# stdstu12/YUME

Measured on NVIDIA H100. Metric: latent_frames_per_sec, higher is better.
Workload: dtype bf16

## Files before the change

yume_b200/csrc/attention.cu:

```cuda
#include "yb_host.h"
#include "yb_ptx.cuh"

namespace yb {

constexpr int ATT_THREADS = 384;
constexpr int ATT_TILE_BYTES = 128 * 128 * 2;

struct AttParams {
  __nv_bfloat16* out;
  long long ldo;
  int Lq, Lk;
  int nkv;
  int accumulate;
  __nv_bfloat16* out_peers[8];
  int sp_world, sp_rank, sp_Lp;
  float scale_log2;
  int nq, full_units, ns;
  float* ws_o;
  float* ws_ml;
};

template <bool P_SMEM>
struct AttCfg {
  static constexpr int NS = P_SMEM ? 4 : 5;
  static constexpr int Q_OFF = 0;
  static constexpr int P_OFF = ATT_TILE_BYTES;
  static constexpr int KV_OFF = P_SMEM ? 2 * ATT_TILE_BYTES : ATT_TILE_BYTES;
  static constexpr int BAR_OFF = KV_OFF + NS * ATT_TILE_BYTES;
  static constexpr int SMEM_BYTES = BAR_OFF + 256 + 1024;
  static_assert(SMEM_BYTES <= 227 * 1024, "shared memory budget");
};

template <bool P_SMEM>
__global__ void __launch_bounds__(ATT_THREADS, 1)
attention_kernel(const __grid_constant__ CUtensorMap tmQ, const __grid_constant__ CUtensorMap tmK,
                 const __grid_constant__ CUtensorMap tmV, const AttParams p) {
  using Cfg = AttCfg<P_SMEM>;
  constexpr int NS = Cfg::NS;
  extern __shared__ uint8_t smem_raw[];
  uint8_t* smem = reinterpret_cast<uint8_t*>((reinterpret_cast<uintptr_t>(smem_raw) + 1023) & ~uintptr_t(1023));
  uint64_t* q_full = reinterpret_cast<uint64_t*>(smem + Cfg::BAR_OFF);
  uint64_t* q_empty = q_full + 1;
  uint64_t* kv_full = q_empty + 1;
  uint64_t* kv_empty = kv_full + NS;

  const int warp = threadIdx.x >> 5;
  const int lane = threadIdx.x & 31;
  int unit = blockIdx.x, kv_begin = 0, nkv = p.nkv;
  if (static_cast<int>(blockIdx.x) >= p.full_units) {
    const int r = blockIdx.x - p.full_units;
    unit = p.full_units + r / p.ns;
    const int per = (((p.nkv + p.ns - 1) / p.ns) + 1) & ~1;
    kv_begin = (r % p.ns) * per;
    nkv = min(per, p.nkv - kv_begin);
  }
  const int head = unit / p.nq;
  const int q0 = (unit - head * p.nq) * 256;
  const int nx = q0 + 128 < p.Lq ? 2 : 1;

  if (threadIdx.x == 0) {
    tma_prefetch_desc(&tmQ);
    tma_prefetch_desc(&tmK);
    tma_prefetch_desc(&tmV);
    mbar_init(q_full, 1);
    mbar_init(q_empty, 8);
    for (int i = 0; i < NS; ++i) {
      mbar_init(&kv_full[i], 1);
      mbar_init(&kv_empty[i], 8);
    }
    fence_barrier_init();
  }
  __syncthreads();

  if (warp < 4) {
    setmaxnreg_dec<40>();
    if (warp == 0 && lane == 0) {
      int it = 0;
      for (int X = 0; X < nx; ++X) {
        if (X == 1) mbar_wait(q_empty, 0);
        mbar_arrive_expect_tx(q_full, ATT_TILE_BYTES);
        for (int s = 0; s < 2; ++s)
          tma_load_2d(smem + Cfg::Q_OFF + s * 16384, &tmQ, q_full, head * 128 + s * 64, q0 + X * 128);
        for (int jj = 0; jj < 2 * nkv; ++jj, ++it) {
          const int slot = it % NS;
          mbar_wait(&kv_empty[slot], ((it / NS) & 1) ^ 1);
          mbar_arrive_expect_tx(&kv_full[slot], ATT_TILE_BYTES);
          const CUtensorMap* tm = (jj & 1) ? &tmV : &tmK;
          uint8_t* dst = smem + Cfg::KV_OFF + slot * ATT_TILE_BYTES;
          const int j = kv_begin + (jj >> 1);
          tma_load_2d(dst, tm, &kv_full[slot], head * 128, j * 128);
          tma_load_2d(dst + 16384, tm, &kv_full[slot], head * 128 + 64, j * 128);
        }
      }
    }
  } else {
    setmaxnreg_inc<232>();
    const int wg = (warp >> 2) - 1;
    const int q4 = lane >> 2, c2 = 2 * (lane & 3);
    const int row_a = wg * 64 + (warp & 3) * 16 + q4;
    const float sc = p.scale_log2;
    const uint32_t sQ = smem_u32(smem + Cfg::Q_OFF) + wg * 64 * 128;
    const uint32_t sP = smem_u32(smem + Cfg::P_OFF) + wg * 16384;
    int it = 0;
    for (int X = 0; X < nx; ++X) {
      mbar_wait(q_full, X);
      float o[64];
#pragma unroll
      for (int i = 0; i < 64; ++i) o[i] = 0.f;
      float m0 = -INFINITY, m1 = -INFINITY, l0 = 0.f, l1 = 0.f;
      for (int j = 0; j < nkv; ++j, it += 2) {
        const int slot_k = it % NS, slot_v = (it + 1) % NS;
        mbar_wait(&kv_full[slot_k], (it / NS) & 1);
        const uint32_t sK = smem_u32(smem + Cfg::KV_OFF + slot_k * ATT_TILE_BYTES);
        float s[64];
#pragma unroll
        for (int i = 0; i < 64; ++i) s[i] = 0.f;
        wgmma_fence();
#pragma unroll
        for (int kk = 0; kk < 8; ++kk) {
          const uint32_t off = (kk >> 2) * 16384 + (kk & 3) * 32;
          wgmma_ss_acc64<0>(s, make_smem_desc_sw128(sQ + off, 16, 1024), make_smem_desc_sw128(sK + off, 16, 1024), kk != 0);
        }
        wgmma_commit();
        wgmma_wait<0>();
        fence_regs(s);
        __syncwarp();
        if (lane == 0) {
          mbar_arrive(&kv_empty[slot_k]);
          if (j == nkv - 1) mbar_arrive(q_empty);
        }
        const int kv_rem = p.Lk - (kv_begin + j) * 128;
        if (kv_rem < 128) {
#pragma unroll
          for (int i = 0; i < 64; ++i)
            if (8 * (i >> 2) + c2 + (i & 1) >= kv_rem) s[i] = -INFINITY;
        }
        float mx0 = -INFINITY, mx1 = -INFINITY;
#pragma unroll
        for (int g = 0; g < 16; ++g) {
          mx0 = fmaxf(mx0, fmaxf(s[4 * g], s[4 * g + 1]));
          mx1 = fmaxf(mx1, fmaxf(s[4 * g + 2], s[4 * g + 3]));
        }
        mx0 = fmaxf(mx0, __shfl_xor_sync(0xffffffffu, mx0, 1));
        mx0 = fmaxf(mx0, __shfl_xor_sync(0xffffffffu, mx0, 2));
        mx1 = fmaxf(mx1, __shfl_xor_sync(0xffffffffu, mx1, 1));
        mx1 = fmaxf(mx1, __shfl_xor_sync(0xffffffffu, mx1, 2));
        const float mn0 = fmaxf(m0, mx0 * sc), mn1 = fmaxf(m1, mx1 * sc);
        const float al0 = fast_exp2(m0 - mn0), al1 = fast_exp2(m1 - mn1);
        m0 = mn0;
        m1 = mn1;
        l0 *= al0;
        l1 *= al1;
#pragma unroll
        for (int g = 0; g < 16; ++g) {
          o[4 * g] *= al0;
          o[4 * g + 1] *= al0;
          o[4 * g + 2] *= al1;
          o[4 * g + 3] *= al1;
        }
        uint32_t pa[8][4];
#pragma unroll
        for (int kk = 0; kk < 8; ++kk) {
          float e[8];
#pragma unroll
          for (int i = 0; i < 8; ++i) e[i] = fast_exp2(s[8 * kk + i] * sc - ((i & 2) ? m1 : m0));
          l0 += (e[0] + e[1]) + (e[4] + e[5]);
          l1 += (e[2] + e[3]) + (e[6] + e[7]);
          pa[kk][0] = pack_bf16x2(e[0], e[1]);
          pa[kk][1] = pack_bf16x2(e[2], e[3]);
          pa[kk][2] = pack_bf16x2(e[4], e[5]);
          pa[kk][3] = pack_bf16x2(e[6], e[7]);
        }
        if (P_SMEM) {
          const int ra = row_a - wg * 64, rb = ra + 8;
#pragma unroll
          for (int kk = 0; kk < 8; ++kk) {
            uint8_t* slab = smem + Cfg::P_OFF + wg * 16384 + (kk >> 2) * 8192;
            const int k0 = (kk & 3) * 16 + c2, k1 = k0 + 8;
            *reinterpret_cast<uint32_t*>(slab + ra * 128 + (((k0 >> 3) ^ (ra & 7)) << 4) + (k0 & 7) * 2) = pa[kk][0];
            *reinterpret_cast<uint32_t*>(slab + rb * 128 + (((k0 >> 3) ^ (rb & 7)) << 4) + (k0 & 7) * 2) = pa[kk][1];
            *reinterpret_cast<uint32_t*>(slab + ra * 128 + (((k1 >> 3) ^ (ra & 7)) << 4) + (k1 & 7) * 2) = pa[kk][2];
            *reinterpret_cast<uint32_t*>(slab + rb * 128 + (((k1 >> 3) ^ (rb & 7)) << 4) + (k1 & 7) * 2) = pa[kk][3];
          }
          fence_proxy_async_smem();
          named_bar_sync(1 + wg, 128);
        }
        mbar_wait(&kv_full[slot_v], ((it + 1) / NS) & 1);
        const uint32_t sV = smem_u32(smem + Cfg::KV_OFF + slot_v * ATT_TILE_BYTES);
        wgmma_fence();
#pragma unroll
        for (int kk = 0; kk < 8; ++kk) {
          const uint64_t vdesc = make_smem_desc_sw128(sV + kk * 2048, 16384, 1024);
          if (P_SMEM)
            wgmma_ss_acc64<1>(o, make_smem_desc_sw128(sP + (kk >> 2) * 8192 + (kk & 3) * 32, 16, 1024), vdesc, 1u);
          else
            wgmma_rs_n128_tb(o, pa[kk], vdesc, 1u);
        }
        wgmma_commit();
        wgmma_wait<0>();
        fence_regs(o);
        __syncwarp();
        if (lane == 0) mbar_arrive(&kv_empty[slot_v]);
      }
      l0 += __shfl_xor_sync(0xffffffffu, l0, 1);
      l0 += __shfl_xor_sync(0xffffffffu, l0, 2);
      l1 += __shfl_xor_sync(0xffffffffu, l1, 1);
      l1 += __shfl_xor_sync(0xffffffffu, l1, 2);

#pragma unroll
      for (int h = 0; h < 2; ++h) {
        const int row_t = X * 128 + row_a + 8 * h;
        const float m = h ? m1 : m0, l = h ? l1 : l0;
        if (static_cast<int>(blockIdx.x) >= p.full_units) {
          const long long prow = static_cast<long long>(blockIdx.x - p.full_units) * 256 + row_t;
          float* wo = p.ws_o + prow * 128;
#pragma unroll
          for (int g = 0; g < 16; ++g) *reinterpret_cast<float2*>(wo + 8 * g + c2) = make_float2(o[4 * g + 2 * h], o[4 * g + 2 * h + 1]);
          if ((lane & 3) == 0) *reinterpret_cast<float2*>(p.ws_ml + prow * 2) = make_float2(m, l);
          continue;
        }
        const int q_row = q0 + row_t;
        if (q_row >= p.Lq) continue;
        __nv_bfloat16* orow = p.out + static_cast<long long>(q_row) * p.ldo + head * 128;
        if (p.sp_world > 1) {
          const int owner = q_row / p.sp_Lp;
          const int t = q_row - owner * p.sp_Lp;
          if (owner < p.sp_world)
            orow = p.out_peers[owner] + (static_cast<long long>(p.sp_rank) * p.sp_Lp + t) * p.ldo + head * 128;
        }
        const float inv = 1.0f / l;
#pragma unroll
        for (int g = 0; g < 16; ++g) {
          uint32_t* dst = reinterpret_cast<uint32_t*>(orow + 8 * g + c2);
          float v0 = o[4 * g + 2 * h] * inv, v1 = o[4 * g + 2 * h + 1] * inv;
          if (p.accumulate) {
            const float2 prev = __bfloat1622float2(*reinterpret_cast<const __nv_bfloat162*>(dst));
            v0 += prev.x;
            v1 += prev.y;
          }
          *dst = pack_bf16x2(v0, v1);
        }
      }
    }
  }
}

__global__ void __launch_bounds__(256) attention_combine_kernel(const AttParams p, int tail_units) {
  const int gw = blockIdx.x * 8 + (threadIdx.x >> 5);
  const int lane = threadIdx.x & 31;
  if (gw >= tail_units * 256) return;
  const int tu = gw >> 8, r = gw & 255;
  const int unit = p.full_units + tu;
  const int head = unit / p.nq;
  const int q_row = (unit - head * p.nq) * 256 + r;
  if (q_row >= p.Lq) return;
  float M = -INFINITY;
  for (int sgm = 0; sgm < p.ns; ++sgm) M = fmaxf(M, p.ws_ml[((static_cast<long long>(tu) * p.ns + sgm) * 256 + r) * 2]);
  float4 acc = make_float4(0.f, 0.f, 0.f, 0.f);
  float lsum = 0.f;
  for (int sgm = 0; sgm < p.ns; ++sgm) {
    const long long prow = (static_cast<long long>(tu) * p.ns + sgm) * 256 + r;
    const float2 ml = *reinterpret_cast<const float2*>(p.ws_ml + prow * 2);
    const float w = exp2f(ml.x - M);
    const float4 o = *reinterpret_cast<const float4*>(p.ws_o + prow * 128 + lane * 4);
    acc.x += o.x * w; acc.y += o.y * w; acc.z += o.z * w; acc.w += o.w * w;
    lsum += ml.y * w;
  }
  const float inv = 1.0f / lsum;
  __nv_bfloat16* orow = p.out + static_cast<long long>(q_row) * p.ldo + head * 128;
  if (p.sp_world > 1) {
    const int owner = q_row / p.sp_Lp;
    const int t = q_row - owner * p.sp_Lp;
    if (owner < p.sp_world)
      orow = p.out_peers[owner] + (static_cast<long long>(p.sp_rank) * p.sp_Lp + t) * p.ldo + head * 128;
  }
  *reinterpret_cast<uint2*>(orow + lane * 4) = make_uint2(pack_bf16x2(acc.x * inv, acc.y * inv), pack_bf16x2(acc.z * inv, acc.w * inv));
}

static void attention_plan(int units, int nkv, int sms, bool allowed, int force_ns, int* full_units, int* tail, int* ns) {
  *full_units = units;
  *tail = 0;
  *ns = 1;
  if (!allowed || force_ns == 1) return;
  if (force_ns >= 2 && nkv >= 2 * force_ns) {
    *tail = units;
    *ns = force_ns;
  } else if (force_ns == 0 && units > sms && units % sms != 0 && 2 * (units % sms) <= sms && nkv >= 16) {
    *tail = units % sms;
    *ns = sms / *tail < 4 ? sms / *tail : 4;
  }
  while (*ns > 1 && (*ns - 1) * ((((nkv + *ns - 1) / *ns) + 1) & ~1) >= nkv) --*ns;
  if (*ns == 1) *tail = 0;
  *full_units = units - *tail;
}

static size_t split_workspace_bytes(size_t ctas) { return ctas * 256 * 130 * sizeof(float); }

static int g_debug_force_split = 0;

template <bool P_SMEM>
static int launch_attention(const CUtensorMap& tmQ, const CUtensorMap& tmK, const CUtensorMap& tmV,
                            AttParams p, int heads, cudaStream_t stream, int force_ns, void* ws, long long ws_bytes) {
  using Cfg = AttCfg<P_SMEM>;
  auto kern = attention_kernel<P_SMEM>;
  static bool attr_set[kMaxDevices] = {false};
  if (int rc = ensure_dynamic_smem(kern, Cfg::SMEM_BYTES, attr_set, "attention")) return rc;
  if (force_ns == 0 && g_debug_force_split >= 1 && g_debug_force_split <= 4) force_ns = g_debug_force_split;
  p.nq = (p.Lq + 255) / 256;
  const int units = p.nq * heads;
  int tail = 0;
  p.ws_o = p.ws_ml = nullptr;
  const bool allowed = !p.accumulate && ws != nullptr;
  attention_plan(units, p.nkv, sm_count(), allowed, force_ns, &p.full_units, &tail, &p.ns);
  if (tail > 0) {
    const size_t ctas = static_cast<size_t>(tail) * p.ns;
    if (ws_bytes < 0 || static_cast<size_t>(ws_bytes) < split_workspace_bytes(ctas) || (reinterpret_cast<uintptr_t>(ws) & 0xF)) {
      p.full_units = units;
      tail = 0;
      p.ns = 1;
    } else {
      p.ws_o = static_cast<float*>(ws);
      p.ws_ml = p.ws_o + ctas * 256 * 128;
    }
  }
  kern<<<p.full_units + tail * p.ns, ATT_THREADS, Cfg::SMEM_BYTES, stream>>>(tmQ, tmK, tmV, p);
  int rc = check_launch("attention");
  if (rc || tail == 0) return rc;
  attention_combine_kernel<<<tail * 32, 256, 0, stream>>>(p, tail);
  return check_launch("attention_combine");
}

static int dispatch_attention(const void* q, long long ldq, const void* k, long long ldk, const void* v, long long ldv,
                              AttParams p, int heads, cudaStream_t stream, int flags, void* ws, long long ws_bytes) {
  const int force_ns = (flags >> YB_ATT_SPLIT_SHIFT) & 7;
  if (force_ns > 4) return YB_ERR_ARG;
  if ((flags >> YB_ATT_EMU_SHIFT) & 3) return YB_ERR_ARG;
  CUtensorMap tmQ, tmK, tmV;
  const uint64_t cols = static_cast<uint64_t>(heads) * 128;
  int rc = make_tmap_bf16_2d(&tmQ, q, p.Lq, cols, ldq, 128, 64);
  if (rc) return rc;
  rc = make_tmap_bf16_2d(&tmK, k, p.Lk, cols, ldk, 128, 64);
  if (rc) return rc;
  rc = make_tmap_bf16_2d(&tmV, v, p.Lk, cols, ldv, 128, 64);
  if (rc) return rc;
  if (flags & YB_ATT_P_SMEM) return launch_attention<true>(tmQ, tmK, tmV, p, heads, stream, force_ns, ws, ws_bytes);
  return launch_attention<false>(tmQ, tmK, tmV, p, heads, stream, force_ns, ws, ws_bytes);
}

}

extern "C" int yb_debug_force_split(int ns) {
  if (ns < 0 || ns > 4) return YB_ERR_ARG;
  yb::g_debug_force_split = ns;
  return YB_OK;
}

extern "C" int yb_attention_plan(int Lq, int Lk, int heads, int sms, int flags, int* out4) {
  if (Lq <= 0 || Lk <= 0 || heads <= 0 || sms <= 0 || !out4) return YB_ERR_ARG;
  int force_ns = (flags >> YB_ATT_SPLIT_SHIFT) & 7;
  if (force_ns > 4) return YB_ERR_ARG;
  if (force_ns == 0 && yb::g_debug_force_split >= 1) force_ns = yb::g_debug_force_split;
  const int nkv = (Lk + 127) / 128;
  int full_units, tail, ns;
  yb::attention_plan(((Lq + 255) / 256) * heads, nkv, sms, !(flags & YB_ATT_ACCUMULATE), force_ns, &full_units, &tail, &ns);
  out4[0] = full_units;
  out4[1] = tail;
  out4[2] = ns;
  out4[3] = ns > 1 ? ((((nkv + ns - 1) / ns) + 1) & ~1) : nkv;
  return YB_OK;
}

extern "C" long long yb_attention_workspace_bytes(int Lq, int Lk, int heads, int sms, int flags) {
  int plan[4];
  if (yb_attention_plan(Lq, Lk, heads, sms, flags, plan)) return -1;
  return static_cast<long long>(yb::split_workspace_bytes(static_cast<size_t>(plan[1]) * plan[2]));
}

extern "C" int yb_attention_ex(const void* q, long long ldq, const void* k, long long ldk, const void* v,
                               long long ldv, void* out, long long ldo, int Lq, int Lk, int heads, float scale,
                               int flags, void* ws, long long ws_bytes, void* trace, void* stream_) {
  using namespace yb;
  if (!q || !k || !v || !out) return YB_ERR_ARG;
  if (Lq <= 0 || Lk <= 0 || heads <= 0) return YB_ERR_ARG;
  if ((ldo % 8) != 0 || (reinterpret_cast<uintptr_t>(out) & 0xF)) return YB_ERR_ALIGNMENT;
  AttParams p;
  p.out = static_cast<__nv_bfloat16*>(out);
  p.ldo = ldo;
  p.Lq = Lq;
  p.Lk = Lk;
  p.nkv = (Lk + 127) / 128;
  p.accumulate = (flags & YB_ATT_ACCUMULATE) ? 1 : 0;
  (void)trace;
  p.sp_world = 1;
  p.sp_rank = 0;
  p.sp_Lp = 0;
  p.scale_log2 = scale * 1.4426950408889634f;
  return dispatch_attention(q, ldq, k, ldk, v, ldv, p, heads, reinterpret_cast<cudaStream_t>(stream_), flags, ws, ws_bytes);
}

extern "C" int yb_attention(const void* q, long long ldq, const void* k, long long ldk, const void* v, long long ldv,
                            void* out, long long ldo, int Lq, int Lk, int heads, float scale, int flags,
                            void* stream_) {
  return yb_attention_ex(q, ldq, k, ldk, v, ldv, out, ldo, Lq, Lk, heads, scale, flags, nullptr, 0, nullptr, stream_);
}

extern "C" int yb_attention_sp(const void* q, long long ldq, const void* k, long long ldk, const void* v, long long ldv,
                               void* const* out_peers, long long ldo, int Lq, int Lk, int heads, float scale, int world,
                               int rank, int Lp, int flags, void* ws, long long ws_bytes, void* stream_) {
  using namespace yb;
  if (!q || !k || !v || !out_peers || world < 2 || world > 8 || rank < 0 || rank >= world || Lp <= 0) return YB_ERR_ARG;
  if (Lq != world * Lp || Lk <= 0 || Lk > Lq || heads <= 0 || (ldo % 8)) return YB_ERR_ARG;
  if (flags & (YB_ATT_ACCUMULATE | YB_ATT_P_SMEM)) return YB_ERR_ARG;
  AttParams p;
  p.out = static_cast<__nv_bfloat16*>(out_peers[rank]);
  p.ldo = ldo;
  p.Lq = Lq;
  p.Lk = Lk;
  p.nkv = (Lk + 127) / 128;
  p.accumulate = 0;
  p.scale_log2 = scale * 1.4426950408889634f;
  for (int i = 0; i < 8; ++i) p.out_peers[i] = i < world ? static_cast<__nv_bfloat16*>(out_peers[i]) : nullptr;
  p.sp_world = world;
  p.sp_rank = rank;
  p.sp_Lp = Lp;
  return dispatch_attention(q, ldq, k, ldk, v, ldv, p, heads, reinterpret_cast<cudaStream_t>(stream_), flags, ws, ws_bytes);
}
```

yume_b200/csrc/yb_ptx.cuh:

```cuda
#pragma once
#include <cstdint>
#include <cstdio>
#include <cuda.h>
#include <cuda_runtime.h>
#include <cuda_bf16.h>

namespace yb {

__device__ __forceinline__ uint32_t smem_u32(const void* p) {
  return static_cast<uint32_t>(__cvta_generic_to_shared(p));
}

template <int N>
__device__ __forceinline__ void setmaxnreg_inc() {
  asm volatile("setmaxnreg.inc.sync.aligned.u32 %0;\n" ::"n"(N));
}
template <int N>
__device__ __forceinline__ void setmaxnreg_dec() {
  asm volatile("setmaxnreg.dec.sync.aligned.u32 %0;\n" ::"n"(N));
}
__device__ __forceinline__ void named_bar_sync(int id, int count) {
  asm volatile("bar.sync %0, %1;" ::"r"(id), "r"(count) : "memory");
}

__device__ __forceinline__ void mbar_init(uint64_t* bar, uint32_t count) {
  asm volatile("mbarrier.init.shared::cta.b64 [%0], %1;" ::"r"(smem_u32(bar)), "r"(count) : "memory");
}
__device__ __forceinline__ void fence_barrier_init() {
  asm volatile("fence.mbarrier_init.release.cluster;" ::: "memory");
}
__device__ __forceinline__ void fence_proxy_async_smem() {
  asm volatile("fence.proxy.async.shared::cta;" ::: "memory");
}
__device__ __forceinline__ void mbar_arrive_expect_tx(uint64_t* bar, uint32_t bytes) {
  asm volatile("mbarrier.arrive.expect_tx.shared::cta.b64 _, [%0], %1;" ::"r"(smem_u32(bar)), "r"(bytes)
               : "memory");
}
__device__ __forceinline__ void mbar_arrive(uint64_t* bar) {
  asm volatile("mbarrier.arrive.shared::cta.b64 _, [%0];" ::"r"(smem_u32(bar)) : "memory");
}
__device__ __forceinline__ bool mbar_try_wait(uint64_t* bar, uint32_t parity) {
  uint32_t ok;
  asm volatile(
      "{\n\t.reg .pred p;\n\t"
      "mbarrier.try_wait.parity.shared::cta.b64 p, [%1], %2;\n\t"
      "selp.u32 %0, 1, 0, p;\n\t}\n"
      : "=r"(ok)
      : "r"(smem_u32(bar)), "r"(parity)
      : "memory");
  return ok != 0;
}
#ifndef YB_WAIT_LIMIT_CYCLES
#define YB_WAIT_LIMIT_CYCLES 8000000000LL
#endif
__device__ __forceinline__ void mbar_wait(uint64_t* bar, uint32_t parity) {
  if (mbar_try_wait(bar, parity)) return;
  const long long t0 = clock64();
  while (!mbar_try_wait(bar, parity)) {
    if (clock64() - t0 > YB_WAIT_LIMIT_CYCLES) {
#ifdef YB_DEBUG_WAIT
      printf("yb: mbarrier wait timeout block=(%d,%d) thread=%d bar=%u parity=%u\n", blockIdx.x, blockIdx.y,
             threadIdx.x, smem_u32(bar), parity);
#endif
      __trap();
    }
  }
}
__device__ __forceinline__ void mbar_wait_cluster(uint64_t* bar, uint32_t parity) {
  const long long t0 = clock64();
  for (;;) {
    uint32_t ok;
    asm volatile(
        "{\n\t.reg .pred p;\n\t"
        "mbarrier.try_wait.parity.acquire.cluster.shared::cta.b64 p, [%1], %2;\n\t"
        "selp.u32 %0, 1, 0, p;\n\t}\n"
        : "=r"(ok)
        : "r"(smem_u32(bar)), "r"(parity)
        : "memory");
    if (ok) return;
    if (clock64() - t0 > YB_WAIT_LIMIT_CYCLES) __trap();
  }
}

__device__ __forceinline__ uint32_t cluster_ctarank() {
  uint32_t r;
  asm volatile("mov.u32 %0, %%cluster_ctarank;" : "=r"(r));
  return r;
}
__device__ __forceinline__ void cluster_sync_all() {
  asm volatile("barrier.cluster.arrive.release.aligned;\n\tbarrier.cluster.wait.acquire.aligned;" ::: "memory");
}
__device__ __forceinline__ void mbar_arrive_cluster(uint64_t* bar, uint32_t cta) {
  uint32_t remote;
  asm volatile("mapa.shared::cluster.u32 %0, %1, %2;" : "=r"(remote) : "r"(smem_u32(bar)), "r"(cta));
  asm volatile("mbarrier.arrive.release.cluster.shared::cluster.b64 _, [%0];" ::"r"(remote) : "memory");
}

__device__ __forceinline__ void tma_prefetch_desc(const CUtensorMap* tmap) {
  asm volatile("prefetch.tensormap [%0];" ::"l"(reinterpret_cast<uint64_t>(tmap)) : "memory");
}
__device__ __forceinline__ void tma_load_2d(void* smem_dst, const CUtensorMap* tmap, uint64_t* bar, int c0, int c1) {
  asm volatile(
      "cp.async.bulk.tensor.2d.shared::cluster.global.tile.mbarrier::complete_tx::bytes [%0], [%1, {%3, %4}], [%2];"
      ::"r"(smem_u32(smem_dst)), "l"(reinterpret_cast<uint64_t>(tmap)), "r"(smem_u32(bar)), "r"(c0), "r"(c1)
      : "memory");
}
__device__ __forceinline__ void tma_load_2d_multicast(void* smem_dst, const CUtensorMap* tmap, uint64_t* bar, int c0, int c1,
                                                      uint16_t mask) {
  asm volatile(
      "cp.async.bulk.tensor.2d.shared::cluster.global.mbarrier::complete_tx::bytes.multicast::cluster [%0], [%1, {%3, %4}], "
      "[%2], %5;" ::"r"(smem_u32(smem_dst)),
      "l"(reinterpret_cast<uint64_t>(tmap)), "r"(smem_u32(bar)), "r"(c0), "r"(c1), "h"(mask)
      : "memory");
}
__device__ __forceinline__ void tma_load_3d(void* smem_dst, const CUtensorMap* tmap, uint64_t* bar, int c0, int c1,
                                            int c2) {
  asm volatile(
      "cp.async.bulk.tensor.3d.shared::cluster.global.tile.mbarrier::complete_tx::bytes [%0], [%1, {%3, %4, %5}], [%2];"
      ::"r"(smem_u32(smem_dst)), "l"(reinterpret_cast<uint64_t>(tmap)), "r"(smem_u32(bar)), "r"(c0), "r"(c1), "r"(c2)
      : "memory");
}
__device__ __forceinline__ void tma_load_4d(void* smem_dst, const CUtensorMap* tmap, uint64_t* bar, int c0, int c1,
                                            int c2, int c3) {
  asm volatile(
      "cp.async.bulk.tensor.4d.shared::cluster.global.tile.mbarrier::complete_tx::bytes [%0], [%1, {%3, %4, %5, %6}], [%2];"
      ::"r"(smem_u32(smem_dst)), "l"(reinterpret_cast<uint64_t>(tmap)), "r"(smem_u32(bar)), "r"(c0), "r"(c1), "r"(c2),
      "r"(c3)
      : "memory");
}

__device__ __forceinline__ uint64_t make_smem_desc_sw128(uint32_t smem_addr, uint32_t lbo_bytes, uint32_t sbo_bytes) {
  uint64_t d = 0;
  d |= static_cast<uint64_t>((smem_addr & 0x3FFFF) >> 4);
  d |= static_cast<uint64_t>((lbo_bytes >> 4) & 0x3FFF) << 16;
  d |= static_cast<uint64_t>((sbo_bytes >> 4) & 0x3FFF) << 32;
  d |= static_cast<uint64_t>(1) << 62;
  return d;
}
__device__ __forceinline__ void wgmma_fence() { asm volatile("wgmma.fence.sync.aligned;" ::: "memory"); }
__device__ __forceinline__ void wgmma_commit() { asm volatile("wgmma.commit_group.sync.aligned;" ::: "memory"); }
template <int N>
__device__ __forceinline__ void wgmma_wait() {
  asm volatile("wgmma.wait_group.sync.aligned %0;" ::"n"(N) : "memory");
}
template <int R>
__device__ __forceinline__ void fence_regs(float (&d)[R]) {
#pragma unroll
  for (int i = 0; i < R; ++i) asm volatile("" : "+f"(d[i])::"memory");
}

template <int OFF>
__device__ __forceinline__ void wgmma_ss_n64(float (&d)[128], uint64_t adesc, uint64_t bdesc, uint32_t accumulate) {
  asm volatile(
      "{\n\t.reg .pred p;\n\t"
      "setp.ne.b32 p, %34, 0;\n\t"
      "wgmma.mma_async.sync.aligned.m64n64k16.f32.bf16.bf16 {%0, %1, %2, %3, %4, %5, %6, %7, %8, %9, %10, %11, %12, %13, %14, %15, %16, %17, %18, %19, %20, %21, %22, %23, %24, %25, %26, %27, %28, %29, %30, %31}, %32, %33, p, 1, 1, 0, 0;\n\t}\n"
      : "+f"(d[OFF + 0]), "+f"(d[OFF + 1]), "+f"(d[OFF + 2]), "+f"(d[OFF + 3]), "+f"(d[OFF + 4]), "+f"(d[OFF + 5]), "+f"(d[OFF + 6]), "+f"(d[OFF + 7]), "+f"(d[OFF + 8]), "+f"(d[OFF + 9]), "+f"(d[OFF + 10]), "+f"(d[OFF + 11]), "+f"(d[OFF + 12]), "+f"(d[OFF + 13]), "+f"(d[OFF + 14]), "+f"(d[OFF + 15]), "+f"(d[OFF + 16]), "+f"(d[OFF + 17]), "+f"(d[OFF + 18]), "+f"(d[OFF + 19]), "+f"(d[OFF + 20]), "+f"(d[OFF + 21]), "+f"(d[OFF + 22]), "+f"(d[OFF + 23]), "+f"(d[OFF + 24]), "+f"(d[OFF + 25]), "+f"(d[OFF + 26]), "+f"(d[OFF + 27]), "+f"(d[OFF + 28]), "+f"(d[OFF + 29]), "+f"(d[OFF + 30]), "+f"(d[OFF + 31])
      : "l"(adesc), "l"(bdesc), "r"(accumulate));
}
template <int OFF>
__device__ __forceinline__ void wgmma_ss_n128(float (&d)[128], uint64_t adesc, uint64_t bdesc, uint32_t accumulate) {
  asm volatile(
      "{\n\t.reg .pred p;\n\t"
      "setp.ne.b32 p, %66, 0;\n\t"
      "wgmma.mma_async.sync.aligned.m64n128k16.f32.bf16.bf16 {%0, %1, %2, %3, %4, %5, %6, %7, %8, %9, %10, %11, %12, %13, %14, %15, %16, %17, %18, %19, %20, %21, %22, %23, %24, %25, %26, %27, %28, %29, %30, %31, %32, %33, %34, %35, %36, %37, %38, %39, %40, %41, %42, %43, %44, %45, %46, %47, %48, %49, %50, %51, %52, %53, %54, %55, %56, %57, %58, %59, %60, %61, %62, %63}, %64, %65, p, 1, 1, 0, 0;\n\t}\n"
      : "+f"(d[OFF + 0]), "+f"(d[OFF + 1]), "+f"(d[OFF + 2]), "+f"(d[OFF + 3]), "+f"(d[OFF + 4]), "+f"(d[OFF + 5]), "+f"(d[OFF + 6]), "+f"(d[OFF + 7]), "+f"(d[OFF + 8]), "+f"(d[OFF + 9]), "+f"(d[OFF + 10]), "+f"(d[OFF + 11]), "+f"(d[OFF + 12]), "+f"(d[OFF + 13]), "+f"(d[OFF + 14]), "+f"(d[OFF + 15]), "+f"(d[OFF + 16]), "+f"(d[OFF + 17]), "+f"(d[OFF + 18]), "+f"(d[OFF + 19]), "+f"(d[OFF + 20]), "+f"(d[OFF + 21]), "+f"(d[OFF + 22]), "+f"(d[OFF + 23]), "+f"(d[OFF + 24]), "+f"(d[OFF + 25]), "+f"(d[OFF + 26]), "+f"(d[OFF + 27]), "+f"(d[OFF + 28]), "+f"(d[OFF + 29]), "+f"(d[OFF + 30]), "+f"(d[OFF + 31]), "+f"(d[OFF + 32]), "+f"(d[OFF + 33]), "+f"(d[OFF + 34]), "+f"(d[OFF + 35]), "+f"(d[OFF + 36]), "+f"(d[OFF + 37]), "+f"(d[OFF + 38]), "+f"(d[OFF + 39]), "+f"(d[OFF + 40]), "+f"(d[OFF + 41]), "+f"(d[OFF + 42]), "+f"(d[OFF + 43]), "+f"(d[OFF + 44]), "+f"(d[OFF + 45]), "+f"(d[OFF + 46]), "+f"(d[OFF + 47]), "+f"(d[OFF + 48]), "+f"(d[OFF + 49]), "+f"(d[OFF + 50]), "+f"(d[OFF + 51]), "+f"(d[OFF + 52]), "+f"(d[OFF + 53]), "+f"(d[OFF + 54]), "+f"(d[OFF + 55]), "+f"(d[OFF + 56]), "+f"(d[OFF + 57]), "+f"(d[OFF + 58]), "+f"(d[OFF + 59]), "+f"(d[OFF + 60]), "+f"(d[OFF + 61]), "+f"(d[OFF + 62]), "+f"(d[OFF + 63])
      : "l"(adesc), "l"(bdesc), "r"(accumulate));
}
template <int OFF>
__device__ __forceinline__ void wgmma_ss_n256(float (&d)[128], uint64_t adesc, uint64_t bdesc, uint32_t accumulate) {
  asm volatile(
      "{\n\t.reg .pred p;\n\t"
      "setp.ne.b32 p, %130, 0;\n\t"
      "wgmma.mma_async.sync.aligned.m64n256k16.f32.bf16.bf16 {%0, %1, %2, %3, %4, %5, %6, %7, %8, %9, %10, %11, %12, %13, %14, %15, %16, %17, %18, %19, %20, %21, %22, %23, %24, %25, %26, %27, %28, %29, %30, %31, %32, %33, %34, %35, %36, %37, %38, %39, %40, %41, %42, %43, %44, %45, %46, %47, %48, %49, %50, %51, %52, %53, %54, %55, %56, %57, %58, %59, %60, %61, %62, %63, %64, %65, %66, %67, %68, %69, %70, %71, %72, %73, %74, %75, %76, %77, %78, %79, %80, %81, %82, %83, %84, %85, %86, %87, %88, %89, %90, %91, %92, %93, %94, %95, %96, %97, %98, %99, %100, %101, %102, %103, %104, %105, %106, %107, %108, %109, %110, %111, %112, %113, %114, %115, %116, %117, %118, %119, %120, %121, %122, %123, %124, %125, %126, %127}, %128, %129, p, 1, 1, 0, 0;\n\t}\n"
      : "+f"(d[OFF + 0]), "+f"(d[OFF + 1]), "+f"(d[OFF + 2]), "+f"(d[OFF + 3]), "+f"(d[OFF + 4]), "+f"(d[OFF + 5]), "+f"(d[OFF + 6]), "+f"(d[OFF + 7]), "+f"(d[OFF + 8]), "+f"(d[OFF + 9]), "+f"(d[OFF + 10]), "+f"(d[OFF + 11]), "+f"(d[OFF + 12]), "+f"(d[OFF + 13]), "+f"(d[OFF + 14]), "+f"(d[OFF + 15]), "+f"(d[OFF + 16]), "+f"(d[OFF + 17]), "+f"(d[OFF + 18]), "+f"(d[OFF + 19]), "+f"(d[OFF + 20]), "+f"(d[OFF + 21]), "+f"(d[OFF + 22]), "+f"(d[OFF + 23]), "+f"(d[OFF + 24]), "+f"(d[OFF + 25]), "+f"(d[OFF + 26]), "+f"(d[OFF + 27]), "+f"(d[OFF + 28]), "+f"(d[OFF + 29]), "+f"(d[OFF + 30]), "+f"(d[OFF + 31]), "+f"(d[OFF + 32]), "+f"(d[OFF + 33]), "+f"(d[OFF + 34]), "+f"(d[OFF + 35]), "+f"(d[OFF + 36]), "+f"(d[OFF + 37]), "+f"(d[OFF + 38]), "+f"(d[OFF + 39]), "+f"(d[OFF + 40]), "+f"(d[OFF + 41]), "+f"(d[OFF + 42]), "+f"(d[OFF + 43]), "+f"(d[OFF + 44]), "+f"(d[OFF + 45]), "+f"(d[OFF + 46]), "+f"(d[OFF + 47]), "+f"(d[OFF + 48]), "+f"(d[OFF + 49]), "+f"(d[OFF + 50]), "+f"(d[OFF + 51]), "+f"(d[OFF + 52]), "+f"(d[OFF + 53]), "+f"(d[OFF + 54]), "+f"(d[OFF + 55]), "+f"(d[OFF + 56]), "+f"(d[OFF + 57]), "+f"(d[OFF + 58]), "+f"(d[OFF + 59]), "+f"(d[OFF + 60]), "+f"(d[OFF + 61]), "+f"(d[OFF + 62]), "+f"(d[OFF + 63]), "+f"(d[OFF + 64]), "+f"(d[OFF + 65]), "+f"(d[OFF + 66]), "+f"(d[OFF + 67]), "+f"(d[OFF + 68]), "+f"(d[OFF + 69]), "+f"(d[OFF + 70]), "+f"(d[OFF + 71]), "+f"(d[OFF + 72]), "+f"(d[OFF + 73]), "+f"(d[OFF + 74]), "+f"(d[OFF + 75]), "+f"(d[OFF + 76]), "+f"(d[OFF + 77]), "+f"(d[OFF + 78]), "+f"(d[OFF + 79]), "+f"(d[OFF + 80]), "+f"(d[OFF + 81]), "+f"(d[OFF + 82]), "+f"(d[OFF + 83]), "+f"(d[OFF + 84]), "+f"(d[OFF + 85]), "+f"(d[OFF + 86]), "+f"(d[OFF + 87]), "+f"(d[OFF + 88]), "+f"(d[OFF + 89]), "+f"(d[OFF + 90]), "+f"(d[OFF + 91]), "+f"(d[OFF + 92]), "+f"(d[OFF + 93]), "+f"(d[OFF + 94]), "+f"(d[OFF + 95]), "+f"(d[OFF + 96]), "+f"(d[OFF + 97]), "+f"(d[OFF + 98]), "+f"(d[OFF + 99]), "+f"(d[OFF + 100]), "+f"(d[OFF + 101]), "+f"(d[OFF + 102]), "+f"(d[OFF + 103]), "+f"(d[OFF + 104]), "+f"(d[OFF + 105]), "+f"(d[OFF + 106]), "+f"(d[OFF + 107]), "+f"(d[OFF + 108]), "+f"(d[OFF + 109]), "+f"(d[OFF + 110]), "+f"(d[OFF + 111]), "+f"(d[OFF + 112]), "+f"(d[OFF + 113]), "+f"(d[OFF + 114]), "+f"(d[OFF + 115]), "+f"(d[OFF + 116]), "+f"(d[OFF + 117]), "+f"(d[OFF + 118]), "+f"(d[OFF + 119]), "+f"(d[OFF + 120]), "+f"(d[OFF + 121]), "+f"(d[OFF + 122]), "+f"(d[OFF + 123]), "+f"(d[OFF + 124]), "+f"(d[OFF + 125]), "+f"(d[OFF + 126]), "+f"(d[OFF + 127])
      : "l"(adesc), "l"(bdesc), "r"(accumulate));
}
__device__ __forceinline__ void wgmma_rs_n128_tb(float (&d)[64], const uint32_t (&a)[4], uint64_t bdesc, uint32_t accumulate) {
  asm volatile(
      "{\n\t.reg .pred p;\n\t"
      "setp.ne.b32 p, %69, 0;\n\t"
      "wgmma.mma_async.sync.aligned.m64n128k16.f32.bf16.bf16 {%0, %1, %2, %3, %4, %5, %6, %7, %8, %9, %10, %11, %12, %13, %14, %15, %16, %17, %18, %19, %20, %21, %22, %23, %24, %25, %26, %27, %28, %29, %30, %31, %32, %33, %34, %35, %36, %37, %38, %39, %40, %41, %42, %43, %44, %45, %46, %47, %48, %49, %50, %51, %52, %53, %54, %55, %56, %57, %58, %59, %60, %61, %62, %63}, {%64, %65, %66, %67}, %68, p, 1, 1, 1;\n\t}\n"
      : "+f"(d[0]), "+f"(d[1]), "+f"(d[2]), "+f"(d[3]), "+f"(d[4]), "+f"(d[5]), "+f"(d[6]), "+f"(d[7]), "+f"(d[8]), "+f"(d[9]), "+f"(d[10]), "+f"(d[11]), "+f"(d[12]), "+f"(d[13]), "+f"(d[14]), "+f"(d[15]), "+f"(d[16]), "+f"(d[17]), "+f"(d[18]), "+f"(d[19]), "+f"(d[20]), "+f"(d[21]), "+f"(d[22]), "+f"(d[23]), "+f"(d[24]), "+f"(d[25]), "+f"(d[26]), "+f"(d[27]), "+f"(d[28]), "+f"(d[29]), "+f"(d[30]), "+f"(d[31]), "+f"(d[32]), "+f"(d[33]), "+f"(d[34]), "+f"(d[35]), "+f"(d[36]), "+f"(d[37]), "+f"(d[38]), "+f"(d[39]), "+f"(d[40]), "+f"(d[41]), "+f"(d[42]), "+f"(d[43]), "+f"(d[44]), "+f"(d[45]), "+f"(d[46]), "+f"(d[47]), "+f"(d[48]), "+f"(d[49]), "+f"(d[50]), "+f"(d[51]), "+f"(d[52]), "+f"(d[53]), "+f"(d[54]), "+f"(d[55]), "+f"(d[56]), "+f"(d[57]), "+f"(d[58]), "+f"(d[59]), "+f"(d[60]), "+f"(d[61]), "+f"(d[62]), "+f"(d[63])
      : "r"(a[0]), "r"(a[1]), "r"(a[2]), "r"(a[3]), "l"(bdesc), "r"(accumulate));
}
template <int TB>
__device__ __forceinline__ void wgmma_ss_acc64(float (&d)[64], uint64_t adesc, uint64_t bdesc, uint32_t accumulate) {
  asm volatile(
      "{\n\t.reg .pred p;\n\t"
      "setp.ne.b32 p, %66, 0;\n\t"
      "wgmma.mma_async.sync.aligned.m64n128k16.f32.bf16.bf16 {%0, %1, %2, %3, %4, %5, %6, %7, %8, %9, %10, %11, %12, %13, %14, %15, %16, %17, %18, %19, %20, %21, %22, %23, %24, %25, %26, %27, %28, %29, %30, %31, %32, %33, %34, %35, %36, %37, %38, %39, %40, %41, %42, %43, %44, %45, %46, %47, %48, %49, %50, %51, %52, %53, %54, %55, %56, %57, %58, %59, %60, %61, %62, %63}, %64, %65, p, 1, 1, 0, %67;\n\t}\n"
      : "+f"(d[0]), "+f"(d[1]), "+f"(d[2]), "+f"(d[3]), "+f"(d[4]), "+f"(d[5]), "+f"(d[6]), "+f"(d[7]), "+f"(d[8]), "+f"(d[9]), "+f"(d[10]), "+f"(d[11]), "+f"(d[12]), "+f"(d[13]), "+f"(d[14]), "+f"(d[15]), "+f"(d[16]), "+f"(d[17]), "+f"(d[18]), "+f"(d[19]), "+f"(d[20]), "+f"(d[21]), "+f"(d[22]), "+f"(d[23]), "+f"(d[24]), "+f"(d[25]), "+f"(d[26]), "+f"(d[27]), "+f"(d[28]), "+f"(d[29]), "+f"(d[30]), "+f"(d[31]), "+f"(d[32]), "+f"(d[33]), "+f"(d[34]), "+f"(d[35]), "+f"(d[36]), "+f"(d[37]), "+f"(d[38]), "+f"(d[39]), "+f"(d[40]), "+f"(d[41]), "+f"(d[42]), "+f"(d[43]), "+f"(d[44]), "+f"(d[45]), "+f"(d[46]), "+f"(d[47]), "+f"(d[48]), "+f"(d[49]), "+f"(d[50]), "+f"(d[51]), "+f"(d[52]), "+f"(d[53]), "+f"(d[54]), "+f"(d[55]), "+f"(d[56]), "+f"(d[57]), "+f"(d[58]), "+f"(d[59]), "+f"(d[60]), "+f"(d[61]), "+f"(d[62]), "+f"(d[63])
      : "l"(adesc), "l"(bdesc), "r"(accumulate), "n"(TB));
}

__device__ __forceinline__ uint32_t pack_bf16x2(float lo, float hi) {
  __nv_bfloat162 v = __floats2bfloat162_rn(lo, hi);
  return *reinterpret_cast<uint32_t*>(&v);
}
__device__ __forceinline__ float fast_exp2(float x) {
  float y;
  asm volatile("ex2.approx.ftz.f32 %0, %1;" : "=f"(y) : "f"(x));
  return y;
}
__device__ __forceinline__ float fast_tanh(float x) {
  float y;
  asm volatile("tanh.approx.f32 %0, %1;" : "=f"(y) : "f"(x));
  return y;
}
__device__ __forceinline__ float gelu_tanh(float x) {
  const float k0 = 0.7978845608028654f, k1 = 0.044715f;
  float u = k0 * (x + k1 * x * x * x);
  return 0.5f * x * (1.0f + fast_tanh(u));
}

}
```

Baseline: 38.83.

## Overlap softmax with next QK GEMM and ping-pong warpgroups in attention

Restructures the consumer loop of the attention kernel in the FA3 style. The S=QK^T GEMM for block j is issued together with the PV GEMM for block j-1, and the softmax of block j runs while the PV GEMM is still in flight. Named barriers make the two consumer warpgroups take turns issuing WGMMAs, so one warpgroup's softmax overlaps the other's tensor-core work. It also moves the trap out of line in mbar_wait to shrink code, at the cost of more live registers and more complex barrier protocols.

Result: faster. 39.83, median of 6 (+2.6%).

```diff
diff --git a/yume_b200/csrc/attention.cu b/yume_b200/csrc/attention.cu
--- a/yume_b200/csrc/attention.cu
+++ b/yume_b200/csrc/attention.cu
@@ -101,107 +101,155 @@
     const float sc = p.scale_log2;
     const uint32_t sQ = smem_u32(smem + Cfg::Q_OFF) + wg * 64 * 128;
     const uint32_t sP = smem_u32(smem + Cfg::P_OFF) + wg * 16384;
-    int it = 0;
-    for (int X = 0; X < nx; ++X) {
+    float o[64], s[64];
+    uint32_t pa[8][4];
+    float m0 = -INFINITY, m1 = -INFINITY, l0 = 0.f, l1 = 0.f;
+
+    auto kv_wait = [&](int i) { mbar_wait(&kv_full[i % NS], (i / NS) & 1); };
+    auto kv_release = [&](int i) {
+      __syncwarp();
+      if (lane == 0) mbar_arrive(&kv_empty[i % NS]);
+    };
+    auto kv_smem = [&](int i) { return smem_u32(smem + Cfg::KV_OFF + (i % NS) * ATT_TILE_BYTES); };
+    auto issue_s = [&](int i) {
+      const uint32_t sK = kv_smem(i);
+#pragma unroll
+      for (int c = 0; c < 64; ++c) s[c] = 0.f;
+      wgmma_fence();
+#pragma unroll
+      for (int kk = 0; kk < 8; ++kk) {
+        const uint32_t off = (kk >> 2) * 16384 + (kk & 3) * 32;
+        wgmma_ss_acc64<0>(s, make_smem_desc_sw128(sQ + off, 16, 1024), make_smem_desc_sw128(sK + off, 16, 1024), kk != 0);
+      }
+      wgmma_commit();
+    };
+    auto issue_pv = [&](int i) {
+      const uint32_t sV = kv_smem(i);
+      wgmma_fence();
+#pragma unroll
+      for (int kk = 0; kk < 8; ++kk) {
+        const uint64_t vdesc = make_smem_desc_sw128(sV + kk * 2048, 16384, 1024);
+        if (P_SMEM)
+          wgmma_ss_acc64<1>(o, make_smem_desc_sw128(sP + (kk >> 2) * 8192 + (kk & 3) * 32, 16, 1024), vdesc, 1u);
+        else
+          wgmma_rs_n128_tb(o, pa[kk], vdesc, 1u);
+      }
+      wgmma_commit();
+    };
+    auto softmax = [&](int j, float& al0, float& al1) {
+      const int kv_rem = p.Lk - (kv_begin + j) * 128;
+      if (kv_rem < 128) {
+#pragma unroll
+        for (int i = 0; i < 64; ++i)
+          if (8 * (i >> 2) + c2 + (i & 1) >= kv_rem) s[i] = -INFINITY;
+      }
+      float mx0 = -INFINITY, mx1 = -INFINITY;
+#pragma unroll
+      for (int g = 0; g < 16; ++g) {
+        mx0 = fmaxf(mx0, fmaxf(s[4 * g], s[4 * g + 1]));
+        mx1 = fmaxf(mx1, fmaxf(s[4 * g + 2], s[4 * g + 3]));
+      }
+      mx0 = fmaxf(mx0, __shfl_xor_sync(0xffffffffu, mx0, 1));
+      mx0 = fmaxf(mx0, __shfl_xor_sync(0xffffffffu, mx0, 2));
+      mx1 = fmaxf(mx1, __shfl_xor_sync(0xffffffffu, mx1, 1));
+      mx1 = fmaxf(mx1, __shfl_xor_sync(0xffffffffu, mx1, 2));
+      const float mn0 = fmaxf(m0, mx0 * sc), mn1 = fmaxf(m1, mx1 * sc);
+      al0 = fast_exp2(m0 - mn0);
+      al1 = fast_exp2(m1 - mn1);
+      m0 = mn0;
+      m1 = mn1;
+      l0 *= al0;
+      l1 *= al1;
+#pragma unroll
+      for (int kk = 0; kk < 8; ++kk) {
+        float* e = s + 8 * kk;
+#pragma unroll
+        for (int i = 0; i < 8; ++i) e[i] = fast_exp2(e[i] * sc - ((i & 2) ? m1 : m0));
+        l0 += (e[0] + e[1]) + (e[4] + e[5]);
+        l1 += (e[2] + e[3]) + (e[6] + e[7]);
+      }
+    };
+    auto rescale_pack = [&](float al0, float al1) {
+#pragma unroll
+      for (int g = 0; g < 16; ++g) {
+        o[4 * g] *= al0;
+        o[4 * g + 1] *= al0;
+        o[4 * g + 2] *= al1;
+        o[4 * g + 3] *= al1;
+      }
+#pragma unroll
+      for (int kk = 0; kk < 8; ++kk) {
+        const float* e = s + 8 * kk;
+        pa[kk][0] = pack_bf16x2(e[0], e[1]);
+        pa[kk][1] = pack_bf16x2(e[2], e[3]);
+        pa[kk][2] = pack_bf16x2(e[4], e[5]);
+        pa[kk][3] = pack_bf16x2(e[6], e[7]);
+      }
+      if (P_SMEM) {
+        const int ra = row_a - wg * 64, rb = ra + 8;
+#pragma unroll
+        for (int kk = 0; kk < 8; ++kk) {
+          uint8_t* slab = smem + Cfg::P_OFF + wg * 16384 + (kk >> 2) * 8192;
+          const int k0 = (kk & 3) * 16 + c2, k1 = k0 + 8;
+          *reinterpret_cast<uint32_t*>(slab + ra * 128 + (((k0 >> 3) ^ (ra & 7)) << 4) + (k0 & 7) * 2) = pa[kk][0];
+          *reinterpret_cast<uint32_t*>(slab + rb * 128 + (((k0 >> 3) ^ (rb & 7)) << 4) + (k0 & 7) * 2) = pa[kk][1];
+          *reinterpret_cast<uint32_t*>(slab + ra * 128 + (((k1 >> 3) ^ (ra & 7)) << 4) + (k1 & 7) * 2) = pa[kk][2];
+          *reinterpret_cast<uint32_t*>(slab + rb * 128 + (((k1 >> 3) ^ (rb & 7)) << 4) + (k1 & 7) * 2) = pa[kk][3];
+        }
+        fence_proxy_async_smem();
+        named_bar_sync(1 + wg, 128);
+      }
+    };
+    auto turn_wait = [&]() { named_bar_sync(3 + wg, 256); };
+    auto turn_pass = [&](bool last) {
+      if (wg == 0 || !last) named_bar_arrive(4 - wg, 256);
+    };
+
+    if (wg == 1) named_bar_arrive(3, 256);
+    int it0 = 0;
+    for (int X = 0; X < nx; ++X, it0 += 2 * nkv) {
       mbar_wait(q_full, X);
-      float o[64];
 #pragma unroll
       for (int i = 0; i < 64; ++i) o[i] = 0.f;
-      float m0 = -INFINITY, m1 = -INFINITY, l0 = 0.f, l1 = 0.f;
-      for (int j = 0; j < nkv; ++j, it += 2) {
-        const int slot_k = it % NS, slot_v = (it + 1) % NS;
-        mbar_wait(&kv_full[slot_k], (it / NS) & 1);
-        const uint32_t sK = smem_u32(smem + Cfg::KV_OFF + slot_k * ATT_TILE_BYTES);
-        float s[64];
-#pragma unroll
-        for (int i = 0; i < 64; ++i) s[i] = 0.f;
-        wgmma_fence();
-#pragma unroll
-        for (int kk = 0; kk < 8; ++kk) {
-          const uint32_t off = (kk >> 2) * 16384 + (kk & 3) * 32;
-          wgmma_ss_acc64<0>(s, make_smem_desc_sw128(sQ + off, 16, 1024), make_smem_desc_sw128(sK + off, 16, 1024), kk != 0);
-        }
-        wgmma_commit();
-        wgmma_wait<0>();
+      m0 = m1 = -INFINITY;
+      l0 = l1 = 0.f;
+      float al0, al1;
+      kv_wait(it0);
+      turn_wait();
+      issue_s(it0);
+      turn_pass(X == nx - 1 && nkv == 1);
+      wgmma_wait<0>();
+      fence_regs(s);
+      kv_release(it0);
+      if (nkv == 1 && lane == 0) mbar_arrive(q_empty);
+      softmax(0, al0, al1);
+      rescale_pack(al0, al1);
+      for (int j = 1; j < nkv; ++j) {
+        const int ik = it0 + 2 * j;
+        kv_wait(ik);
+        kv_wait(ik - 1);
+        turn_wait();
+        issue_s(ik);
+        issue_pv(ik - 1);
+        turn_pass(X == nx - 1 && j == nkv - 1);
+        wgmma_wait<1>();
         fence_regs(s);
-        __syncwarp();
-        if (lane == 0) {
-          mbar_arrive(&kv_empty[slot_k]);
-          if (j == nkv - 1) mbar_arrive(q_empty);
-        }
-        const int kv_rem = p.Lk - (kv_begin + j) * 128;
-        if (kv_rem < 128) {
-#pragma unroll
-          for (int i = 0; i < 64; ++i)
-            if (8 * (i >> 2) + c2 + (i & 1) >= kv_rem) s[i] = -INFINITY;
-        }
-        float mx0 = -INFINITY, mx1 = -INFINITY;
-#pragma unroll
-        for (int g = 0; g < 16; ++g) {
-          mx0 = fmaxf(mx0, fmaxf(s[4 * g], s[4 * g + 1]));
-          mx1 = fmaxf(mx1, fmaxf(s[4 * g + 2], s[4 * g + 3]));
-        }
-        mx0 = fmaxf(mx0, __shfl_xor_sync(0xffffffffu, mx0, 1));
-        mx0 = fmaxf(mx0, __shfl_xor_sync(0xffffffffu, mx0, 2));
-        mx1 = fmaxf(mx1, __shfl_xor_sync(0xffffffffu, mx1, 1));
-        mx1 = fmaxf(mx1, __shfl_xor_sync(0xffffffffu, mx1, 2));
-        const float mn0 = fmaxf(m0, mx0 * sc), mn1 = fmaxf(m1, mx1 * sc);
-        const float al0 = fast_exp2(m0 - mn0), al1 = fast_exp2(m1 - mn1);
-        m0 = mn0;
-        m1 = mn1;
-        l0 *= al0;
-        l1 *= al1;
-#pragma unroll
-        for (int g = 0; g < 16; ++g) {
-          o[4 * g] *= al0;
-          o[4 * g + 1] *= al0;
-          o[4 * g + 2] *= al1;
-          o[4 * g + 3] *= al1;
-        }
-        uint32_t pa[8][4];
-#pragma unroll
-        for (int kk = 0; kk < 8; ++kk) {
-          float e[8];
-#pragma unroll
-          for (int i = 0; i < 8; ++i) e[i] = fast_exp2(s[8 * kk + i] * sc - ((i & 2) ? m1 : m0));
-          l0 += (e[0] + e[1]) + (e[4] + e[5]);
-          l1 += (e[2] + e[3]) + (e[6] + e[7]);
-          pa[kk][0] = pack_bf16x2(e[0], e[1]);
-          pa[kk][1] = pack_bf16x2(e[2], e[3]);
-          pa[kk][2] = pack_bf16x2(e[4], e[5]);
-          pa[kk][3] = pack_bf16x2(e[6], e[7]);
-        }
-        if (P_SMEM) {
-          const int ra = row_a - wg * 64, rb = ra + 8;
-#pragma unroll
-          for (int kk = 0; kk < 8; ++kk) {
-            uint8_t* slab = smem + Cfg::P_OFF + wg * 16384 + (kk >> 2) * 8192;
-            const int k0 = (kk & 3) * 16 + c2, k1 = k0 + 8;
-            *reinterpret_cast<uint32_t*>(slab + ra * 128 + (((k0 >> 3) ^ (ra & 7)) << 4) + (k0 & 7) * 2) = pa[kk][0];
-            *reinterpret_cast<uint32_t*>(slab + rb * 128 + (((k0 >> 3) ^ (rb & 7)) << 4) + (k0 & 7) * 2) = pa[kk][1];
-            *reinterpret_cast<uint32_t*>(slab + ra * 128 + (((k1 >> 3) ^ (ra & 7)) << 4) + (k1 & 7) * 2) = pa[kk][2];
-            *reinterpret_cast<uint32_t*>(slab + rb * 128 + (((k1 >> 3) ^ (rb & 7)) << 4) + (k1 & 7) * 2) = pa[kk][3];
-          }
-          fence_proxy_async_smem();
-          named_bar_sync(1 + wg, 128);
-        }
-        mbar_wait(&kv_full[slot_v], ((it + 1) / NS) & 1);
-        const uint32_t sV = smem_u32(smem + Cfg::KV_OFF + slot_v * ATT_TILE_BYTES);
-        wgmma_fence();
-#pragma unroll
-        for (int kk = 0; kk < 8; ++kk) {
-          const uint64_t vdesc = make_smem_desc_sw128(sV + kk * 2048, 16384, 1024);
-          if (P_SMEM)
-            wgmma_ss_acc64<1>(o, make_smem_desc_sw128(sP + (kk >> 2) * 8192 + (kk & 3) * 32, 16, 1024), vdesc, 1u);
-          else
-            wgmma_rs_n128_tb(o, pa[kk], vdesc, 1u);
-        }
-        wgmma_commit();
+        kv_release(ik);
+        if (j == nkv - 1 && lane == 0) mbar_arrive(q_empty);
+        softmax(j, al0, al1);
         wgmma_wait<0>();
         fence_regs(o);
-        __syncwarp();
-        if (lane == 0) mbar_arrive(&kv_empty[slot_v]);
-      }
+#pragma unroll
+        for (int kk = 0; kk < 8; ++kk) fence_regs(pa[kk]);
+        kv_release(ik - 1);
+        rescale_pack(al0, al1);
+      }
+      const int iv = it0 + 2 * nkv - 1;
+      kv_wait(iv);
+      issue_pv(iv);
+      wgmma_wait<0>();
+      fence_regs(o);
+      kv_release(iv);
       l0 += __shfl_xor_sync(0xffffffffu, l0, 1);
       l0 += __shfl_xor_sync(0xffffffffu, l0, 2);
       l1 += __shfl_xor_sync(0xffffffffu, l1, 1);
diff --git a/yume_b200/csrc/yb_ptx.cuh b/yume_b200/csrc/yb_ptx.cuh
--- a/yume_b200/csrc/yb_ptx.cuh
+++ b/yume_b200/csrc/yb_ptx.cuh
@@ -53,6 +53,7 @@
 #ifndef YB_WAIT_LIMIT_CYCLES
 #define YB_WAIT_LIMIT_CYCLES 8000000000LL
 #endif
+static __device__ __noinline__ void wait_timeout_trap() { __trap(); }
 __device__ __forceinline__ void mbar_wait(uint64_t* bar, uint32_t parity) {
   if (mbar_try_wait(bar, parity)) return;
   const long long t0 = clock64();
@@ -62,7 +63,7 @@
       printf("yb: mbarrier wait timeout block=(%d,%d) thread=%d bar=%u parity=%u\n", blockIdx.x, blockIdx.y,
              threadIdx.x, smem_u32(bar), parity);
 #endif
-      __trap();
+      wait_timeout_trap();
     }
   }
 }
@@ -194,6 +195,15 @@
       : "l"(adesc), "l"(bdesc), "r"(accumulate), "n"(TB));
 }
 
+__device__ __forceinline__ void named_bar_arrive(int id, int count) {
+  asm volatile("bar.arrive %0, %1;" ::"r"(id), "r"(count) : "memory");
+}
+template <int R>
+__device__ __forceinline__ void fence_regs(uint32_t (&a)[R]) {
+#pragma unroll
+  for (int i = 0; i < R; ++i) asm volatile("" : "+r"(a[i])::"memory");
+}
+
 __device__ __forceinline__ uint32_t pack_bf16x2(float lo, float hi) {
   __nv_bfloat162 v = __floats2bfloat162_rn(lo, hi);
   return *reinterpret_cast<uint32_t*>(&v);
```
